# risc0/paritytech-bn

Hardware: AMD Instinct MI355X
Metric: BN254 pairings/sec (batched) at 1/2/4/8 MI355X; bit-exact vs CPU ref (higher is better)
Workload: dtype u32 (9x29-bit Montgomery digits, integer only)

## Files before the change

include/bn254mi.h:

```cpp
#ifndef BN254MI_H
#define BN254MI_H
#include <stddef.h>
#include <stdint.h>

#ifdef __cplusplus
extern "C" {
#endif

typedef struct { uint64_t l[4]; } bn_fq;
typedef struct { bn_fq c0, c1; } bn_fq2;
typedef struct { uint64_t l[4]; } bn_fr;
typedef struct { bn_fq x, y, z; } bn_g1;
typedef struct { bn_fq2 x, y, z; } bn_g2;
typedef struct { bn_fq c[12]; } bn_gt;

typedef enum {
    BN_OK = 0,
    BN_ERR_INVALID_ARGUMENT = 1,
    BN_ERR_TO_AFFINE = 2,
    BN_ERR_FE_ZERO = 3,
    BN_ERR_HIP = 4,
    BN_ERR_NO_DEVICE = 5,
    BN_ERR_INTERNAL = 6
} bn_status;
// ... 89 lines not shown

int bn_fq_from_slice_many(bn_ctx* ctx, const uint8_t* be32, size_t n, bn_fq* out, uint8_t* status);
int bn_fq_to_big_endian_many(bn_ctx* ctx, const bn_fq* a, size_t n, uint8_t* be32);
int bn_fq2_from_slice_many(bn_ctx* ctx, const uint8_t* be64, size_t n, bn_fq2* out, uint8_t* status);
int bn_fr_from_slice_many(bn_ctx* ctx, const uint8_t* be32, size_t n, bn_fr* out);
int bn_fr_to_big_endian_many(bn_ctx* ctx, const bn_fr* a, size_t n, uint8_t* be32);
int bn_fq_sqrt_many(bn_ctx* ctx, const bn_fq* a, size_t n, bn_fq* out, uint8_t* ok);
int bn_fq2_sqrt_many(bn_ctx* ctx, const bn_fq2* a, size_t n, bn_fq2* out, uint8_t* ok);
int bn_g1_affine_new_many(bn_ctx* ctx, const bn_fq* x, const bn_fq* y, size_t n, bn_g1* out, uint8_t* status);
int bn_g2_affine_new_many(bn_ctx* ctx, const bn_fq2* x, const bn_fq2* y, size_t n, bn_g2* out, uint8_t* status);
int bn_g2_affine_new_many_dev(bn_ctx* ctx, const bn_fq2* d_x, const bn_fq2* d_y, size_t n, bn_g2* d_out,
                              uint8_t* d_status, void* stream);
int bn_g1_from_compressed_many(bn_ctx* ctx, const uint8_t* b33, size_t n, bn_g1* out, uint8_t* status);
int bn_g2_from_compressed_many(bn_ctx* ctx, const uint8_t* b65, size_t n, bn_g2* out, uint8_t* status);
int bn_g1_from_compressed_many_dev(bn_ctx* ctx, const uint8_t* d_b33, size_t n, bn_g1* d_out, uint8_t* d_status,
                                   void* stream);
int bn_g2_from_compressed_many_dev(bn_ctx* ctx, const uint8_t* d_b65, size_t n, bn_g2* d_out, uint8_t* d_status,
                                   void* stream);
int bn_gt_pow_many(bn_ctx* ctx, const bn_gt* a, const bn_fr* k, size_t n, bn_gt* out);
int bn_gt_pow_many_dev(bn_ctx* ctx, const bn_gt* d_a, const bn_fr* d_k, size_t n, bn_gt* d_out, void* stream);

int bn_set_phase_timing(bn_ctx* ctx, int enable);
int bn_set_fe_wide_max(bn_ctx* ctx, size_t n);
int bn_set_latency_max(bn_ctx* ctx, size_t n);
int bn_get_phase_times(bn_ctx* ctx, float ms[4], int* launches);

size_t bn_workspace_bytes(size_t n);
int bn_reserve(bn_ctx* ctx, size_t n);

#ifdef __cplusplus
}
#endif
#endif
```

paritytech-bn_amd/csrc/capi.hip:

```cpp
#include <hip/hip_runtime.h>
#include <stdlib.h>
#include <string.h>

#include <algorithm>
#include <array>
#include <initializer_list>
#include <mutex>
#include <string>
#include <thread>
#include <vector>

#include "kernels.h"

using namespace bn;

#include "ctx.h"

namespace {

int fail(bn_ctx* c, int code, const std::string& msg) {
    if (c) c->err = msg;
    return code;
}
#define HIPCHK(ctx, x)                                                                   \
// ... 1153 lines not shown
        HIPCHK(c, hipGetLastError());
    }
    return BN_OK;
}
int bn_pairing_batch_dev(bn_ctx* c, const bn_g1* d_p, const bn_g2* d_q, size_t n, bn_gt* d_out, int* d_status,
                         void* stream) {
    CTX_GUARD(c);
    return batch_dev(c, d_p, d_q, n, d_out, d_status, 0, pick(c, stream));
}
int bn_miller_loop_batch_dev(bn_ctx* c, const bn_g2* d_q, const bn_g1* d_p, size_t n, bn_gt* d_out, int* d_status,
                             void* stream) {
    CTX_GUARD(c);
    return batch_dev(c, d_p, d_q, n, d_out, d_status, 1, pick(c, stream));
}
int bn_set_latency_max(bn_ctx* c, size_t n) {
    if (c && !c->subs.empty()) {
        for (bn_ctx* d : c->subs) RET_IF(bn_set_latency_max(d, n));
        return BN_OK;
    }
    CTX_GUARD(c);
    c->latency_max = n;
    return BN_OK;
}
int bn_set_fe_wide_max(bn_ctx* c, size_t n) {
    if (c && !c->subs.empty()) {
        for (bn_ctx* d : c->subs) RET_IF(bn_set_fe_wide_max(d, n));
        return BN_OK;
    }
    CTX_GUARD(c);
    c->fe_wide_max = n;
    return BN_OK;
}

int bn_final_exponentiation_many(bn_ctx* c, const bn_gt* f, size_t n, bn_gt* out, uint8_t* ok) {
    if (c && !c->subs.empty()) return bn_multi_final_exponentiation_many(c, f, n, out, ok);
    CTX_GUARD_HOST(c);
    if (n == 0) return BN_OK;
    if (!f || !out) return fail(c, BN_ERR_INVALID_ARGUMENT, "null buffer");
    RET_IF(clear_err(c, c->stream));
    int zero = 0;
    return final_exp_host(c, f, n, out, ok, &zero);
}

int bn_miller_loop_many(bn_ctx* c, const bn_g1* p, const bn_g2* q, size_t n, bn_gt* out) {
    if (c && !c->subs.empty()) return bn_multi_miller_loop_many(c, p, q, n, out);
    CTX_GUARD_HOST(c);
// ... 266 lines not shown
        bn_gt* dout = db + m;
        uint32_t* dprog = (uint32_t*)(dout + m);
        HIPCHK(c, hipMemcpyAsync(da, a + off, m * sizeof(bn_gt), hipMemcpyHostToDevice, c->stream));
        k_gt_load<<<grid_for(kPathLanes * m), kBlock, 0, c->stream>>>(da, m, c->slots + (size_t)1 * kSlotWords * m);
        if (op == BN_FQ12_MUL) {
            HIPCHK(c, hipMemcpyAsync(db, b + off, m * sizeof(bn_gt), hipMemcpyHostToDevice, c->stream));
            k_gt_load<<<grid_for(kPathLanes * m), kBlock, 0, c->stream>>>(db, m, c->slots + (size_t)2 * kSlotWords * m);
        }
        Prog P;
        P.next = 3;
        uint32_t res = P.tmp();
        switch (op) {
            case BN_FQ12_MUL: P.op(OP_MUL, res, 1, 2); break;
            case BN_FQ12_SQR: P.op(OP_SQR, res, 1); break;
            case BN_FQ12_INV: P.op(OP_INV, res, 1); break;
            case BN_FQ12_CYC_SQR: P.op(OP_CYC, res, 1); break;
            case BN_FQ12_EXP_BY_NEG_Z: res = P.exp_by_neg_z(1); break;
            case BN_FQ12_FROB1: P.op(OP_FROB1, res, 1); break;
            case BN_FQ12_FROB2: P.op(OP_FROB2, res, 1); break;
            default: P.op(OP_FROB3, res, 1); break;
        }
        P.finalize({res});
        HIPCHK(c, hipMemcpyAsync(dprog, P.s.data(), P.s.size() * 4, hipMemcpyHostToDevice, c->stream));
        k_fq12_vm<<<grid_pair(kPathLanes * m), kPairBlock, 0, c->stream>>>(dprog, P.steps(), c->slots, m);
        k_gt_store<<<grid_for(kPathLanes * m), kBlock, 0, c->stream>>>(c->slots + (size_t)res * kSlotWords * m, m, m, dout);
        HIPCHK(c, hipGetLastError());
        HIPCHK(c, hipMemcpyAsync(out + off, dout, m * sizeof(bn_gt), hipMemcpyDeviceToHost, c->stream));
        HIPCHK(c, hipStreamSynchronize(c->stream));
    }
    return BN_OK;
}

int bn_fq_from_slice_many(bn_ctx* c, const uint8_t* be32, size_t n, bn_fq* out, uint8_t* st) {
    CTX_GUARD_HOST(c);
    return staged(c, n, {{be32, 32}}, {{out, sizeof(bn_fq)}, {st, 1}}, [&](void** d, size_t m, hipStream_t s) -> int {
        KL(k_fq_from_slice, (const uint8_t*)d[0], m, (bn_fq*)d[1], (uint8_t*)d[2]);
        return BN_OK;
    });
}
int bn_fq_to_big_endian_many(bn_ctx* c, const bn_fq* a, size_t n, uint8_t* be32) {
    CTX_GUARD_HOST(c);
    return staged(c, n, {{a, sizeof(bn_fq)}}, {{be32, 32}}, [&](void** d, size_t m, hipStream_t s) -> int {
        KL(k_fq_to_be, (const bn_fq*)d[0], m, (uint8_t*)d[1]);
        return BN_OK;
    });
}
int bn_fq2_from_slice_many(bn_ctx* c, const uint8_t* be64, size_t n, bn_fq2* out, uint8_t* st) {
// ... 219 lines not shown
```

paritytech-bn_amd/csrc/ctx.h:

```cpp
#pragma once
#include <hip/hip_runtime.h>

#include <array>
#include <mutex>
#include <string>
#include <vector>

#include "../../include/bn254mi.h"

struct bn_ctx {
    int device = 0;
    hipStream_t stream = nullptr;
    std::mutex mu;
    std::mutex err_mu;
    std::string err;
    size_t cap = 0;
    uint32_t* coeffs = nullptr;
    uint32_t* paff = nullptr;
    uint32_t* slots = nullptr;
    uint8_t* flags = nullptr;
    uint32_t* d_prog = nullptr;
    bool timing = false;
    std::vector<hipEvent_t> ev_pool;
    std::vector<std::array<hipEvent_t, 5>> ev_marks;
    int fe_steps = 0;
    int fe_out = 0;
    bool fe_last_out = false;
    size_t fe_wide_max = 0;
    int miller_form = 3;
    size_t latency_max = 0;
    bool latency_w2 = true;
    size_t lat_w1_max = 2048;
    size_t prepare_wide_max = 0;
    int* d_err = nullptr;
    uint32_t* tail_ws = nullptr;
    uint32_t tail_epoch = 0;
    uint32_t* fe_ds_ws = nullptr;
    size_t fe_ds_max = 0;
    size_t stage_bytes = 0;
    void* stage = nullptr;
    int host_pipeline = 1;
    size_t host_piece = 0;
    size_t pin_bytes = 0;
    void* pin = nullptr;
    hipStream_t h2d = nullptr, d2h = nullptr;
    hipEvent_t ev_in[2] = {}, ev_comp[2] = {}, ev_out[2] = {};
    hipEvent_t ws_event = nullptr;
    bool ws_pending = false;
    int msm_window = 0;
    size_t msm_min = 0;
    uint32_t* msm_keys = nullptr;
// ... 29 lines not shown
```

paritytech-bn_amd/csrc/kernels.h:

```cpp
#pragma once
#include <hip/hip_runtime.h>

#include "../../include/bn254mi.h"
#include "pairing.h"
#include "msm.h"

namespace bn {

constexpr int kBlock = 256;
constexpr int kPathLanes = BN_PATH_SPLIT ? 2 : 1;
constexpr int kSlotLaneWords = BN_SPLIT ? 54 : 108;
#if BN_SPLIT
#define BN_PATH_ATTR __attribute__((amdgpu_waves_per_eu(2, 2)))
#else
#define BN_PATH_ATTR
#endif
constexpr int kCoeffFq = BN_NUM_COEFFS * 6;
constexpr size_t kChunk = size_t(1) << 18;
constexpr int kSlotWords = 108;
constexpr int kGtPowEntries = 17;
constexpr uint32_t kMsmSegment = 16;
constexpr int kMsmScanBlock = 1024;

template <int B>
// ... 403 lines not shown
__global__ void __launch_bounds__(kBlock) k_horner_wide(const uint32_t* __restrict__ g, size_t n, SegPlan plan,
                                                        int do_fe, bn_gt* __restrict__ out, int* __restrict__ err, int duo);
__global__ void __launch_bounds__(kBlock) k_horner_tree(const uint32_t* __restrict__ g, SegPlan plan, int do_fe,
                                                        bn_gt* __restrict__ out, int* __restrict__ err, int duo);
__global__ void __launch_bounds__(kPairBlock) k_prepare(const bn_g1* __restrict__ p, const bn_g2* __restrict__ q, size_t n,
                          uint32_t* __restrict__ coeffs, uint32_t* __restrict__ paff, uint8_t* __restrict__ flags,
                          int* __restrict__ err, int mode, int scale);
constexpr int kPrepareWideLanes = 8;
#ifndef BN_LINES_PRESCALED
#define BN_LINES_PRESCALED 1
#endif
__global__ void __launch_bounds__(kPairBlock) k_prepare_wide(const bn_g1* __restrict__ p, const bn_g2* __restrict__ q,
                                                         size_t n, uint32_t* __restrict__ coeffs,
                                                         uint32_t* __restrict__ paff, uint8_t* __restrict__ flags,
                                                         int* __restrict__ err, int mode, int scale);
__global__ void __launch_bounds__(kBlock) k_coeffs_store(const uint32_t* __restrict__ coeffs, size_t n,
                                                         bn_fq2* __restrict__ out);
__global__ void __launch_bounds__(kPairBlock) k_pairing_fused(const bn_g1* __restrict__ p, const bn_g2* __restrict__ q,
                                                          size_t n, uint8_t* __restrict__ flags, int* __restrict__ err,
                                                          int mode, uint32_t* __restrict__ f_out);
__global__ void __launch_bounds__(kBlock) k_miller(const uint32_t* __restrict__ coeffs, const uint32_t* __restrict__ paff,
                         const uint8_t* __restrict__ flags, size_t n, uint32_t* __restrict__ f_out);
__global__ void __launch_bounds__(kPairBlock) k_fq12_vm(const uint32_t* __restrict__ prog, int nsteps, uint32_t* slots, size_t n);
__global__ void __launch_bounds__(kPairBlock) k_pairing_full(const bn_g1* __restrict__ p, const bn_g2* __restrict__ q,
                                                          size_t n, const uint32_t* __restrict__ prog, int nsteps,
                                                          uint32_t* __restrict__ slots, bn_gt* __restrict__ out,
                                                          int* __restrict__ err);
__global__ void __launch_bounds__(kBlock) k_fe_out(const uint32_t* __restrict__ slots, size_t n, int out_slot, const uint8_t* __restrict__ flags,
                         bn_gt* __restrict__ out, uint8_t* __restrict__ ok, int* __restrict__ err);
__global__ void __launch_bounds__(kBlock) k_fe_wide(const uint32_t* __restrict__ f, size_t stride, size_t n,
                                                    bn_gt* __restrict__ out, uint8_t* __restrict__ ok,
                                                    int* __restrict__ err, int duo);
__global__ void __launch_bounds__(kBlock) k_fq12_reduce_wide(const uint32_t* __restrict__ in, size_t in_stride,
                                                             SetSpan sets, uint32_t* __restrict__ out,
                                                             size_t out_stride, size_t out_base, size_t out_set, int per_group);
constexpr int kTailBlock = 256;
__global__ void __launch_bounds__(kTailBlock) k_horner_tree2(const uint32_t* __restrict__ g, SegPlan plan, int do_fe,
                                                             bn_gt* __restrict__ out, int* __restrict__ err,
                                                             const uint32_t* __restrict__ zf);
constexpr int kTailChanWords = 1024 + 2 * 128 * 88;
__global__ void __launch_bounds__(kTailBlock) k_seg_fe1(uint32_t* __restrict__ g, SegPlan plan,
                                                        uint32_t* __restrict__ zf);
constexpr int kTailWsWords = kTailChanWords + 2 * kMaxSeg * 256;
__global__ void __launch_bounds__(kTailBlock) k_seg_tail(const uint32_t* __restrict__ g, SegPlan plan,
                                                         bn_gt* __restrict__ out, int* __restrict__ err,
                                                         uint32_t* __restrict__ ws, uint32_t epoch);
// ... 57 lines not shown
```

paritytech-bn_amd/csrc/kernels_pairing.hip:

```cpp
#ifndef BN_FOLD_LDS
#define BN_FOLD_LDS 1
#endif
#include "fq.h"
#define BN_SPLIT BN_PATH_SPLIT
#include "kernels.h"
#include "lines_wide.h"
#include "fe_vm.h"

namespace bn {

__global__ void BN_PATH_ATTR __launch_bounds__(kPairBlock) k_prepare(const bn_g1* __restrict__ p,
                                                                    const bn_g2* __restrict__ q, size_t n,
                                                                    uint32_t* __restrict__ coeffs,
                                                                    uint32_t* __restrict__ paff,
                                                                    uint8_t* __restrict__ flags,
                                                                    int* __restrict__ err, int mode, int scale) {
    fold_table_init();
    const Balance bal = balance_init();
    const size_t l = lane_id(), i = l / kL, nl = kL * n;
    if (i >= n) return;
    const PairAffine a = pair_to_affine(p, q, i, l, flags, err, mode);
    st_fq(paff, nl, l, 0, a.px);
    st_fq(paff, nl, l, 1, a.py);
    const bool sc = BN_LINES_PRESCALED && scale;
// ... 99 lines not shown
    const size_t l = lane_id(), i = l / kL, nl = kL * n;
    if (i >= n) return;
#pragma unroll 1
    for (int k = 0; k < BN_NUM_COEFFS; ++k)
#pragma unroll
        for (int j = 0; j < 3; ++j) st_ref2(out[(i * BN_NUM_COEFFS + k) * 3 + j], ld_fq2<kLine>(coeffs, nl, l, k * 6 + 2 * j));
}

__global__ void BN_PATH_ATTR __launch_bounds__(kPairBlock) k_pairing_fused(const bn_g1* __restrict__ p,
                                                                          const bn_g2* __restrict__ q, size_t n,
                                                                          uint8_t* __restrict__ flags,
                                                                          int* __restrict__ err, int mode,
                                                                          uint32_t* __restrict__ f_out) {
    fold_table_init();
    const Balance bal = balance_init();
    const size_t l = lane_id(), i = l / kL, nl = kL * n;
    if (i >= n) return;
    const PairAffine a = pair_to_affine(p, q, i, l, flags, err, mode);
    Fq12<kF> f = miller_fused(a.qa, a.px, a.py, [&](int d) { balance_step(bal, (uint32_t)d); });
    if (flags[l]) f = widen<kF>(fq12_one());
    st_fq12(f_out, nl, l, f);
}

__global__ void BN_PATH_ATTR __launch_bounds__(kPairBlock) k_pairing_full(const bn_g1* __restrict__ p,
                                                                         const bn_g2* __restrict__ q, size_t n,
                                                                         const uint32_t* __restrict__ prog, int nsteps,
                                                                         uint32_t* __restrict__ slots,
                                                                         bn_gt* __restrict__ out, int* __restrict__ err) {
    fold_table_init();
    const Balance bal = balance_init();
    const size_t l = lane_id(), i = l / kL, nl = kL * n;
    if (i >= n) return;
    const PairAffine a = pair_to_affine(p, q, i, l, nullptr, err, 0);
    Fq12<kF> f = miller_fused(a.qa, a.px, a.py, [&](int d) { balance_step(bal, (uint32_t)d); });
    if (a.skip) f = widen<kF>(fq12_one());
    const bool zero = !a.skip && fq12_is_zero(f);
    st_fq12(slots, nl, l, f);
    const Fq12<kF> r = fq12_vm_run(prog, nsteps, slots, nl, l, bal, 1u << 20, false);
    if (zero) {
        if ((l % kL) == 0) err_or(err, BN_ERR_FE_ZERO);
        st_gt_zero(out[i]);
    } else if (a.skip) {
        st_gt(out[i], fq12_one());
    } else {
        st_gt(out[i], r);
    }
// ... 141 lines not shown
```

paritytech-bn_amd/csrc/pairing.h:

```cpp
#pragma once
#include "curve.h"

namespace bn {

constexpr int kF = 2;
template <int S, int B>
BN_INLINE Fq12<S> narrow12(const Fq12<B>& a) {
    if constexpr (kv(B) <= S) {
        return widen<S>(fq12_norm(a));
    } else {
        return widen<S>(fq12_fold(a));
    }
}

template <int B, typename Emit>
BN_INLINE void g2_precompute(const G2Aff<B>& q, Emit&& emit) {
    G2Proj r = {widen<kPt>(q.x), widen<kPt>(q.y), widen<kPt>(fq2_one())};
    const G2Aff<B> q_neg = {q.x, fq2_neg(q.y)};
    int k = 0;
#pragma unroll 1
    for (int i = 0; i < BN_NAF_DIGITS; ++i) {
        emit(k++, doubling_step(r));
        if ((kNafNonzero >> i) & 1u) {
            const bool minus = (kNafMinus >> i) & 1u;
            G2Aff<B> base = {q.x, fq2_select(minus, q_neg.y, q.y)};
            emit(k++, mixed_addition_step(r, base));
        }
    }
    G2Aff<kPt> q1 = mul_by_q(q);
    G2Aff<kPt> q2 = mul_by_q(q1);
    q2.y = fq2_neg(q2.y);
    emit(k++, mixed_addition_step(r, q1));
    emit(k++, mixed_addition_step(r, q2));
}

#if BN_SPLIT
#ifndef BN_DOT6_ASM
#define BN_DOT6_ASM 1
#endif
struct LineOps {
    Fq<kLine> y;
    Fq<8> w;
};
template <int X>
BN_INLINE LineOps line_ops(const Fq2<X>& v_in) {
    const Fq<kv(X)> v = fq_norm(v_in.c);
    const bool odd = lane_odd();
#if defined(__HIP_DEVICE_COMPILE__)
    Fq<kjoin(kv(X), kenc(kv(X) + 1, 2))> w;
    dpp_sel_own_partner(w.v, v.v, fq_neg_lazy(v).v);
    (void)odd;
    return {widen<kLine>(fq_bcast_c0(v)), widen<8>(fq_norm(w))};
#else
    const Fq<kv(X)> pv = fq_partner(v);
    return {widen<kLine>(fq_select(odd, pv, v)), widen<8>(fq_norm(fq_pick(odd, v, fq_neg_lazy(pv))))};
#endif
}
BN_INLINE void acc_mad2(Acc& t, const Fq<2>& u, const LineOps& v) {
    acc_mad(t, u, v.y);
    acc_mad(t, fq_partner(u), v.w);
}
template <int F, int X>
BN_INLINE Fq12<2> fq12_mul_by_024_lazy(const Fq12<F>& f_in, const Fq2<X>& x0_in, const Fq2<X>& x4_in,
                                       const Fq2<X>& x2_in) {
    static_assert(kl(F) == 1 && kv(F) <= 2, "fq12_mul_by_024_lazy: f normalized, bound 2");
    const LineOps x0 = line_ops(x0_in), x4 = line_ops(x4_in), x2 = line_ops(x2_in);
    const Fq<2> f0 = widen<2>(f_in.c0.c0.c), f1 = widen<2>(f_in.c1.c0.c), f2 = widen<2>(f_in.c0.c1.c);
    const Fq<2> f3 = widen<2>(f_in.c1.c1.c), f4 = widen<2>(f_in.c0.c2.c), f5 = widen<2>(f_in.c1.c2.c);
    auto xi = [](const Fq<2>& u) { return fq2_fold(fq2_mul_xi(Fq2<2>{u})).c; };
    auto out = [&](const Fq<2>& a, const LineOps& va, const Fq<2>& b, const LineOps& vb, const Fq<2>& c,
                   const LineOps& vc) {
#if BN_DOT6_ASM && BN_DOT2_ASM && defined(__HIP_DEVICE_COMPILE__)
        const Fq<2> pa = fq_partner(a), pb = fq_partner(b), pc = fq_partner(c);
        Fq<2> r;
        asm(BN_ASM_DOT6 : BN_ASM_OUT9(r.v)
            : BN_ASM_IN9(a.v), BN_ASM_IN9(va.y.v), BN_ASM_IN9(pa.v), BN_ASM_IN9(va.w.v), BN_ASM_IN9(b.v),
              BN_ASM_IN9(vb.y.v), BN_ASM_IN9(pb.v), BN_ASM_IN9(vb.w.v), BN_ASM_IN9(c.v), BN_ASM_IN9(vc.y.v),
              BN_ASM_IN9(pc.v), BN_ASM_IN9(vc.w.v), BN_ASM_P
            : BN_ASM_CLOBBER);
        return Fq2<2>{r};
#else
        Acc t = {};
        acc_mad2(t, a, va);
        acc_mad2(t, b, vb);
        acc_mad2(t, c, vc);
        return Fq2<2>{acc_redc<2>(t)};
#endif
    };
    const Fq2<2> o5 = out(f5, x0, f2, x4, f1, x2);
    const Fq2<2> o4 = out(f4, x0, f1, x4, f0, x2);
    const Fq<2> g5 = xi(f5);
    const Fq2<2> o3 = out(f3, x0, f0, x4, g5, x2);
    const Fq<2> g4 = xi(f4);
    const Fq2<2> o2 = out(f2, x0, g5, x4, g4, x2);
    const Fq<2> g3 = xi(f3);
    const Fq2<2> o1 = out(f1, x0, g4, x4, g3, x2);
    const Fq<2> g2 = xi(f2);
    const Fq2<2> o0 = out(f0, x0, g3, x4, g2, x2);
    return {{o0, o2, o4}, {o1, o3, o5}};
}
#endif

template <int B, int PB>
BN_INLINE Fq12<kF> apply_line(const Fq12<B>& f, const Ell& c, const Fq<PB>& px, const Fq<PB>& py) {
#if BN_SPLIT
    return widen<kF>(fq12_mul_by_024_lazy(narrow12<2>(f), c.ell_0, narrow<kLine>(fq2_scale(c.ell_vw, py)),
                                          narrow<kLine>(fq2_scale(c.ell_vv, px))));
#else
    return narrow12<kF>(fq12_mul_by_024(f, c.ell_0, narrow<kLine>(fq2_scale(c.ell_vw, py)),
                                        narrow<kLine>(fq2_scale(c.ell_vv, px))));
// ... 147 lines not shown
```

paritytech-bn_amd/csrc/tower.h:

```cpp
#pragma once
#include "fq.h"


namespace bn {

constexpr int cmax(int a, int b) { return a > b ? a : b; }

constexpr int kInvRounds = 19;
constexpr Limbs9 kR3 = {{0x0e2312b2u, 0x16c05ca2u, 0x0bc84389u, 0x1cdf310bu, 0x11adafddu, 0x032e568eu, 0x1d6ae48cu,
                         0x10d4cd1fu, 0x0026c2d2u}};
BN_INLINE uint32_t bgcd_lin_exact(const uint32_t (&x)[9], const uint32_t (&y)[9], int32_t f, int32_t g,
                                  uint32_t (&r)[9]) {
    int64_t c = 0;
#pragma unroll
    for (int i = 0; i < 9; ++i) {
        const int64_t t = (int64_t)(int32_t)x[i] * f + (int64_t)(int32_t)y[i] * g + c;
        if (i) r[i - 1] = (uint32_t)t & M29;
        c = t >> 29;
    }
    r[8] = (uint32_t)c;
    const uint32_t m = (uint32_t)((int32_t)r[8] >> 31);
    int64_t cn = 0;
#pragma unroll
    for (int i = 0; i < 8; ++i) {
// ... 507 lines not shown
}
template <int L, int B>
BN_INLINE auto pre(const Fq6<B>& a) {
    if constexpr (kv(B) <= L) return a; else return fq6_fold(a);
}
template <int B>
BN_INLINE auto fq6_mul_by_nonresidue(const Fq6<B>& a) { return mk6(fq2_mul_xi(a.c2), a.c0, a.c1); }

template <int A, int B>
BN_INLINE auto fq6_mul(const Fq6<A>& a, const Fq6<B>& b) {
    if constexpr (kv(A) > 20 || kv(B) > 20) return fq6_mul(pre<20>(a), pre<20>(b)); else {
    const auto p1 = fq2_mul2(a.c0, b.c0, a.c1, b.c1);
    const auto& a_a = p1.a;
    const auto& b_b = p1.b;
    const auto p2 = fq2_mul2(a.c2, b.c2, fq2_add(a.c1, a.c2), fq2_add(b.c1, b.c2));
    const auto& c_c = p2.a;
    auto t0 = fq2_sub(fq2_sub(p2.b, b_b), c_c);
    const auto p3 = fq2_mul2(fq2_add(a.c0, a.c1), fq2_add(b.c0, b.c1), fq2_add(a.c0, a.c2), fq2_add(b.c0, b.c2));
    auto t1 = fq2_sub(fq2_sub(p3.a, a_a), b_b);
    auto t2 = fq2_sub(p3.b, a_a);
    return mk6(fq2_add(fq2_mul_xi(t0), a_a), fq2_add(t1, fq2_mul_xi(c_c)), fq2_sub(fq2_add(t2, b_b), c_c));
    }
}
template <int A>
BN_INLINE auto fq6_sqr(const Fq6<A>& a) {
    if constexpr (kv(A) > 20) return fq6_sqr(fq6_fold(a)); else {
    auto s0 = fq2_sqr(a.c0);
    auto s1 = fq2_dbl(fq2_mul(a.c0, a.c1));
    auto s2 = fq2_sqr(fq2_add(fq2_sub(a.c0, a.c1), a.c2));
    auto s3 = fq2_dbl(fq2_mul(a.c1, a.c2));
    auto s4 = fq2_sqr(a.c2);
    return mk6(fq2_add(s0, fq2_mul_xi(s3)), fq2_add(s1, fq2_mul_xi(s4)),
               fq2_sub(fq2_sub(fq2_add(fq2_add(s1, s2), s3), s0), s4));
    }
}
template <int B>
BN_INLINE auto fq6_inv(const Fq6<B>& a_in) {
    auto a = fq6_fold(a_in);
    auto c0 = fq2_fold(fq2_sub(fq2_sqr(a.c0), fq2_mul(a.c1, fq2_mul_xi(a.c2))));
    auto c1 = fq2_fold(fq2_sub(fq2_mul_xi(fq2_sqr(a.c2)), fq2_mul(a.c0, a.c1)));
    auto c2 = fq2_fold(fq2_sub(fq2_sqr(a.c1), fq2_mul(a.c0, a.c2)));
    auto t = fq2_inv(fq2_fold(fq2_add(fq2_mul_xi(fq2_add(fq2_mul(a.c2, c1), fq2_mul(a.c1, c2))), fq2_mul(a.c0, c0))));
    return mk6(fq2_mul(t, c0), fq2_mul(t, c1), fq2_mul(t, c2));
}

BN_INLINE Fq2<1> fq6_frob_c1(int n) {
// ... 29 lines not shown
BN_INLINE Fq12<1> fq12_one() { return {fq6_one(), fq6_zero()}; }
template <int B>
BN_INLINE Fq12<2> fq12_fold(const Fq12<B>& a) { return {fq6_fold(a.c0), fq6_fold(a.c1)}; }
template <int B>
BN_INLINE Fq12<kv(B)> fq12_norm(const Fq12<B>& a) { return {fq6_norm(a.c0), fq6_norm(a.c1)}; }
template <int B>
BN_INLINE bool fq12_is_zero(const Fq12<B>& a) { return ((unsigned)fq6_is_zero(a.c0) & (unsigned)fq6_is_zero(a.c1)) != 0; }
template <int L, int B>
BN_INLINE auto pre(const Fq12<B>& a) {
    if constexpr (kv(B) <= L) return a; else return fq12_fold(a);
}
template <int B>
BN_INLINE auto fq12_conj(const Fq12<B>& a) { return mk12(a.c0, fq6_neg(a.c1)); }
template <int A, int B>
BN_INLINE auto fq12_add(const Fq12<A>& a, const Fq12<B>& b) { return mk12(fq6_add(a.c0, b.c0), fq6_add(a.c1, b.c1)); }
template <int A, int B>
BN_INLINE auto fq12_sub(const Fq12<A>& a, const Fq12<B>& b) { return mk12(fq6_sub(a.c0, b.c0), fq6_sub(a.c1, b.c1)); }
template <int B>
BN_INLINE auto fq12_neg(const Fq12<B>& a) { return mk12(fq6_neg(a.c0), fq6_neg(a.c1)); }

template <int A, int B>
BN_INLINE auto fq12_mul(const Fq12<A>& a, const Fq12<B>& b) {
    if constexpr (kv(A) > 10 || kv(B) > 10) return fq12_mul(pre<10>(a), pre<10>(b)); else {
    auto aa = fq6_fold(fq6_mul(a.c0, b.c0));
    auto bb = fq6_fold(fq6_mul(a.c1, b.c1));
    auto t = fq6_mul(fq6_add(a.c0, a.c1), fq6_add(b.c0, b.c1));
    return mk12(fq6_add(fq6_mul_by_nonresidue(bb), aa), fq6_sub(fq6_sub(t, aa), bb));
    }
}
template <int A>
BN_INLINE auto fq12_sqr(const Fq12<A>& a) {
    if constexpr (kv(A) > 2) return fq12_sqr(fq12_fold(a)); else {
    auto ab = fq6_fold(fq6_mul(a.c0, a.c1));
    auto t = fq6_mul(fq6_add(fq6_mul_by_nonresidue(a.c1), a.c0), fq6_add(a.c0, a.c1));
    return mk12(fq6_sub(fq6_sub(t, ab), fq6_mul_by_nonresidue(ab)), fq6_add(ab, ab));
    }
}
template <int B>
BN_INLINE auto fq12_inv(const Fq12<B>& a_in) {
    auto a = fq12_fold(a_in);
    auto t = fq6_inv(fq6_sub(fq6_fold(fq6_sqr(a.c0)), fq6_mul_by_nonresidue(fq6_fold(fq6_sqr(a.c1)))));
    return mk12(fq6_mul(a.c0, t), fq6_neg(fq6_mul(a.c1, t)));
}
template <int POWER, int B>
BN_INLINE auto fq12_frobenius_map(const Fq12<B>& a) {
    auto c1 = fq6_frobenius_map<POWER>(a.c1);
    if constexpr (POWER == 2) {
        const Fq<1> k = fq_from_limbs<1>(Limbs9{BN_FQ12_C1_2_C0});
        return mk12(fq6_frobenius_map<POWER>(a.c0), mk6(fq2_scale(c1.c0, k), fq2_scale(c1.c1, k), fq2_scale(c1.c2, k)));
    } else {
        Fq2<1> k = fq12_frob_c1(POWER);
        return mk12(fq6_frobenius_map<POWER>(a.c0), mk6(fq2_mul(c1.c0, k), fq2_mul(c1.c1, k), fq2_mul(c1.c2, k)));
    }
}

template <int F, int X>
BN_INLINE auto fq12_mul_by_024(const Fq12<F>& f, const Fq2<X>& ell_0, const Fq2<X>& ell_vw, const Fq2<X>& ell_vv) {
// ... 115 lines not shown
```

paritytech-bn_amd/substrate_bn/_native.py:

```python
import ctypes
import os

import numpy as np

PKG_DIR = os.path.dirname(os.path.dirname(os.path.abspath(__file__)))
LIB_PATH = os.environ.get("BN254MI_LIB") or os.path.join(PKG_DIR, "libbn254mi.so")

BN_OK = 0
BN_ERR_INVALID_ARGUMENT = 1
BN_ERR_TO_AFFINE = 2
BN_ERR_FE_ZERO = 3
BN_ERR_HIP = 4
BN_ERR_NO_DEVICE = 5
BN_ERR_INTERNAL = 6

FQ12_OPS = {"mul": 0, "sqr": 1, "inv": 2, "cyc_sqr": 3, "exp_by_neg_z": 4, "frob1": 5, "frob2": 6, "frob3": 7}

EXPORTS = [
    "bn_ctx_create", "bn_ctx_destroy", "bn_last_error", "bn_ctx_stream",
    "bn_pairing_many", "bn_pairing_many_dev", "bn_pairing_batch", "bn_miller_loop_batch",
    "bn_final_exponentiation_many", "bn_miller_loop_many",
    "bn_g1_mul_many", "bn_g1_mul_many_dev", "bn_g2_mul_many", "bn_g2_mul_many_dev",
    "bn_fq12_op_many", "bn_workspace_bytes", "bn_reserve", "bn_set_phase_timing", "bn_get_phase_times",
    "bn_fq_from_slice_many", "bn_fq_to_big_endian_many", "bn_fq2_from_slice_many", "bn_fr_from_slice_many",
    "bn_fr_to_big_endian_many", "bn_fq_sqrt_many", "bn_fq2_sqrt_many", "bn_g1_affine_new_many",
    "bn_g2_affine_new_many", "bn_g2_affine_new_many_dev", "bn_g1_from_compressed_many", "bn_g2_from_compressed_many",
    "bn_g1_from_compressed_many_dev", "bn_g2_from_compressed_many_dev", "bn_gt_pow_many", "bn_gt_pow_many_dev",
    "bn_ctx_create_multi", "bn_ctx_num_devices", "bn_ctx_device", "bn_shard_range", "bn_pairing_many_allgather_dev",
    "bn_pairing_batch_dev", "bn_miller_loop_batch_dev", "bn_set_fe_wide_max", "bn_g2_precompute_many",
    "bn_set_latency_max", "bn_dev_status",
    "bn_g1_msm", "bn_g1_msm_dev", "bn_set_msm_window", "bn_set_msm_min", "bn_msm_reserve",
] + ["bn_%s_%s_many%s" % (g, op, dev) for g in ("g1", "g2") for op in ("add", "sub", "neg", "normalize", "eq")
     for dev in ("", "_dev")]
GROUP_OPS = ("add", "sub", "neg", "normalize", "eq")

ST_OK, ST_FIELD_INVALID_SLICE_LENGTH, ST_FIELD_INVALID_U512, ST_FIELD_NOT_MEMBER = 0, 1, 2, 3
ST_CURVE_INVALID_ENCODING, ST_CURVE_NOT_MEMBER, ST_GROUP_NOT_ON_CURVE, ST_GROUP_NOT_IN_SUBGROUP = 4, 5, 6, 7


class BnError(RuntimeError):
    def __init__(self, code, msg):
        super().__init__("bn254mi error %d: %s" % (code, msg))
        self.code = code


_lib = None


def load():
    global _lib
    if _lib is not None:
        return _lib
    if not os.path.exists(LIB_PATH):
# ... 30 lines not shown
        "bn_fq2_from_slice_many": ([vp, vp, sz, vp, vp], i),
        "bn_fr_from_slice_many": ([vp, vp, sz, vp], i),
        "bn_fr_to_big_endian_many": ([vp, vp, sz, vp], i),
        "bn_fq_sqrt_many": ([vp, vp, sz, vp, vp], i),
        "bn_fq2_sqrt_many": ([vp, vp, sz, vp, vp], i),
        "bn_g1_affine_new_many": ([vp, vp, vp, sz, vp, vp], i),
        "bn_g2_affine_new_many": ([vp, vp, vp, sz, vp, vp], i),
        "bn_g2_affine_new_many_dev": ([vp, vp, vp, sz, vp, vp, vp], i),
        "bn_g1_from_compressed_many": ([vp, vp, sz, vp, vp], i),
        "bn_g2_from_compressed_many": ([vp, vp, sz, vp, vp], i),
        "bn_g1_from_compressed_many_dev": ([vp, vp, sz, vp, vp, vp], i),
        "bn_g2_from_compressed_many_dev": ([vp, vp, sz, vp, vp, vp], i),
        "bn_gt_pow_many": ([vp, vp, vp, sz, vp], i),
        "bn_gt_pow_many_dev": ([vp, vp, vp, sz, vp, vp], i),
        "bn_ctx_create_multi": ([vp, i, ctypes.POINTER(vp)], i),
        "bn_ctx_num_devices": ([vp], i),
        "bn_ctx_device": ([vp, i], vp),
        "bn_shard_range": ([sz, i, i, ctypes.POINTER(sz), ctypes.POINTER(sz)], None),
        "bn_pairing_many_allgather_dev": ([vp, vp, vp, sz, vp, vp], i),
        "bn_pairing_batch_dev": ([vp, vp, vp, sz, vp, vp, vp], i),
        "bn_miller_loop_batch_dev": ([vp, vp, vp, sz, vp, vp, vp], i),
        "bn_set_fe_wide_max": ([vp, sz], i),
        "bn_set_latency_max": ([vp, sz], i),
        "bn_g2_precompute_many": ([vp, vp, sz, vp], i),
        "bn_dev_status": ([vp, vp], i),
        "bn_g1_msm": ([vp, vp, vp, sz, vp], i),
        "bn_g1_msm_dev": ([vp, vp, vp, sz, vp, vp], i),
        "bn_set_msm_window": ([vp, i], i),
        "bn_set_msm_min": ([vp, sz], i),
        "bn_msm_reserve": ([vp, sz], i),
    }
    for g in ("g1", "g2"):
        for op in GROUP_OPS:
            unary = op in ("neg", "normalize")
            sig["bn_%s_%s_many" % (g, op)] = ([vp, vp, sz, vp] if unary else [vp, vp, vp, sz, vp], i)
            sig["bn_%s_%s_many_dev" % (g, op)] = ([vp, vp, sz, vp, vp] if unary else [vp, vp, vp, sz, vp, vp], i)
    ab_build = bool(os.environ.get("BN254MI_LIB"))
    for name, (args, res) in sig.items():
        if ab_build and not hasattr(L, name):
            continue
        fn = getattr(L, name)
        fn.argtypes = args
        fn.restype = res
    _lib = L
    return L

# ... 191 lines not shown
        self._check(self._L.bn_g2_mul_many_dev(self._h, d_p, d_k, n, d_out, stream))

    def g1_msm_dev(self, d_p, d_k, n, d_out, stream=None):
        self._check(self._L.bn_g1_msm_dev(self._h, d_p, d_k, n, d_out, stream))

    def set_msm_window(self, c):
        self._check(self._L.bn_set_msm_window(self._h, c))

    def set_msm_min(self, n):
        self._check(self._L.bn_set_msm_min(self._h, n))

    def msm_reserve(self, n):
        self._check(self._L.bn_msm_reserve(self._h, n))

    def pairing_batch_dev(self, d_p, d_q, n, d_out, d_status=None, stream=None):
        self._check(self._L.bn_pairing_batch_dev(self._h, d_p, d_q, n, d_out, d_status, stream))

    def miller_loop_batch_dev(self, d_q, d_p, n, d_out, d_status=None, stream=None):
        self._check(self._L.bn_miller_loop_batch_dev(self._h, d_q, d_p, n, d_out, d_status, stream))

    def set_fe_wide_max(self, n):
        self._check(self._L.bn_set_fe_wide_max(self._h, n))

    def set_latency_max(self, n):
        self._check(self._L.bn_set_latency_max(self._h, n))

    def set_phase_timing(self, enable=True):
        self._check(self._L.bn_set_phase_timing(self._h, 1 if enable else 0))

    def phase_times(self):
        ms = np.zeros(4, np.float32)
        cnt = np.zeros(1, np.int32)
        self._check(self._L.bn_get_phase_times(self._h, _ptr(ms), _ptr(cnt)))
        return ms.astype(float), int(cnt[0])

    def _bytes_in(self, b, width):
        b = np.ascontiguousarray(b, dtype=np.uint8)
        if b.size % width:
            raise ValueError("byte buffer of %d is not a multiple of %d" % (b.size, width))
        return b.reshape(-1, width)

    def fq_from_slice_many(self, be32):
        b = self._bytes_in(be32, 32)
        out = np.zeros((b.shape[0], 4), np.uint64)
        st = np.zeros(b.shape[0], np.uint8)
        self._check(self._L.bn_fq_from_slice_many(self._h, _ptr(b), b.shape[0], _ptr(out), _ptr(st)))
# ... 97 lines not shown
```

Baseline: 9.174 million.

## Add lazy Fq6 multiplication via dot6 line-op products for Fq12 mul/sqr

Introduces a lazy Fq6 product that precomputes partner and xi-scaled digits of one operand and forms each output coefficient with a single fused 6-term dot product and one Montgomery reduction. Fq12 mul and sqr in the pairing compilation unit use it by default (BN_FQ6_LAZY=3), replacing the Karatsuba Fq6 multiply with fold steps. The aim is fewer reductions and folds per Fq12 op in the Miller loop and final exponentiation, at the cost of more register pressure from the precomputed operands. It also adds an opt-in pairing-path VM kernel for the fq12 op API, which is off by default.

```diff
diff --git a/include/bn254mi.h b/include/bn254mi.h
--- a/include/bn254mi.h
+++ b/include/bn254mi.h
@@ -135,6 +135,7 @@
 
 int bn_set_phase_timing(bn_ctx* ctx, int enable);
 int bn_set_fe_wide_max(bn_ctx* ctx, size_t n);
+int bn_set_fq12_op_unit(bn_ctx* ctx, int unit);
 int bn_set_latency_max(bn_ctx* ctx, size_t n);
 int bn_get_phase_times(bn_ctx* ctx, float ms[4], int* launches);
 
diff --git a/paritytech-bn_amd/csrc/capi.hip b/paritytech-bn_amd/csrc/capi.hip
--- a/paritytech-bn_amd/csrc/capi.hip
+++ b/paritytech-bn_amd/csrc/capi.hip
@@ -1199,6 +1199,16 @@
     c->latency_max = n;
     return BN_OK;
 }
+int bn_set_fq12_op_unit(bn_ctx* c, int unit) {
+    if (c && !c->subs.empty()) {
+        for (bn_ctx* d : c->subs) RET_IF(bn_set_fq12_op_unit(d, unit));
+        return BN_OK;
+    }
+    CTX_GUARD(c);
+    if (unit != 0 && unit != 1) return fail(c, BN_ERR_INVALID_ARGUMENT, "unit must be 0 or 1");
+    c->fq12_op_unit = unit;
+    return BN_OK;
+}
 int bn_set_fe_wide_max(bn_ctx* c, size_t n) {
     if (c && !c->subs.empty()) {
         for (bn_ctx* d : c->subs) RET_IF(bn_set_fe_wide_max(d, n));
@@ -1511,7 +1521,10 @@
         }
         P.finalize({res});
         HIPCHK(c, hipMemcpyAsync(dprog, P.s.data(), P.s.size() * 4, hipMemcpyHostToDevice, c->stream));
-        k_fq12_vm<<<grid_pair(kPathLanes * m), kPairBlock, 0, c->stream>>>(dprog, P.steps(), c->slots, m);
+        if (c->fq12_op_unit == 1)
+            k_fq12_vm_pairing<<<grid_pair(kPathLanes * m), kPairBlock, 0, c->stream>>>(dprog, P.steps(), c->slots, m);
+        else
+            k_fq12_vm<<<grid_pair(kPathLanes * m), kPairBlock, 0, c->stream>>>(dprog, P.steps(), c->slots, m);
         k_gt_store<<<grid_for(kPathLanes * m), kBlock, 0, c->stream>>>(c->slots + (size_t)res * kSlotWords * m, m, m, dout);
         HIPCHK(c, hipGetLastError());
         HIPCHK(c, hipMemcpyAsync(out + off, dout, m * sizeof(bn_gt), hipMemcpyDeviceToHost, c->stream));
diff --git a/paritytech-bn_amd/csrc/ctx.h b/paritytech-bn_amd/csrc/ctx.h
--- a/paritytech-bn_amd/csrc/ctx.h
+++ b/paritytech-bn_amd/csrc/ctx.h
@@ -27,6 +27,7 @@
     int fe_out = 0;
     bool fe_last_out = false;
     size_t fe_wide_max = 0;
+    int fq12_op_unit = 0;
     int miller_form = 3;
     size_t latency_max = 0;
     bool latency_w2 = true;
diff --git a/paritytech-bn_amd/csrc/kernels.h b/paritytech-bn_amd/csrc/kernels.h
--- a/paritytech-bn_amd/csrc/kernels.h
+++ b/paritytech-bn_amd/csrc/kernels.h
@@ -449,6 +449,7 @@
 __global__ void __launch_bounds__(kBlock) k_miller(const uint32_t* __restrict__ coeffs, const uint32_t* __restrict__ paff,
                          const uint8_t* __restrict__ flags, size_t n, uint32_t* __restrict__ f_out);
 __global__ void __launch_bounds__(kPairBlock) k_fq12_vm(const uint32_t* __restrict__ prog, int nsteps, uint32_t* slots, size_t n);
+__global__ void __launch_bounds__(kPairBlock) k_fq12_vm_pairing(const uint32_t* __restrict__ prog, int nsteps, uint32_t* slots, size_t n);
 __global__ void __launch_bounds__(kPairBlock) k_pairing_full(const bn_g1* __restrict__ p, const bn_g2* __restrict__ q,
                                                           size_t n, const uint32_t* __restrict__ prog, int nsteps,
                                                           uint32_t* __restrict__ slots, bn_gt* __restrict__ out,
diff --git a/paritytech-bn_amd/csrc/kernels_pairing.hip b/paritytech-bn_amd/csrc/kernels_pairing.hip
--- a/paritytech-bn_amd/csrc/kernels_pairing.hip
+++ b/paritytech-bn_amd/csrc/kernels_pairing.hip
@@ -1,5 +1,15 @@
 #ifndef BN_FOLD_LDS
 #define BN_FOLD_LDS 1
+#endif
+#ifndef BN_FQ6_LAZY
+#define BN_FQ6_LAZY 3
+#endif
+#ifndef BN_CYC_LIN
+#if BN_FQ6_LAZY == 3
+#define BN_CYC_LIN 7
+#else
+#define BN_CYC_LIN 0
+#endif
 #endif
 #include "fq.h"
 #define BN_SPLIT BN_PATH_SPLIT
@@ -145,6 +155,15 @@
     st_fq12(f_out, nl, l, f);
 }
 
+__global__ void BN_PATH_ATTR __launch_bounds__(kPairBlock) k_fq12_vm_pairing(const uint32_t* __restrict__ prog,
+                                                                            int nsteps, uint32_t* slots, size_t n) {
+    fold_table_init();
+    const Balance bal = balance_init();
+    const size_t i = lane_id();
+    if (i >= kL * n) return;
+    (void)fq12_vm_run(prog, nsteps, slots, kL * n, i, bal, 0, true);
+}
+
 __global__ void BN_PATH_ATTR __launch_bounds__(kPairBlock) k_pairing_full(const bn_g1* __restrict__ p,
                                                                          const bn_g2* __restrict__ q, size_t n,
                                                                          const uint32_t* __restrict__ prog, int nsteps,
diff --git a/paritytech-bn_amd/csrc/pairing.h b/paritytech-bn_amd/csrc/pairing.h
--- a/paritytech-bn_amd/csrc/pairing.h
+++ b/paritytech-bn_amd/csrc/pairing.h
@@ -35,30 +35,11 @@
 }
 
 #if BN_SPLIT
-#ifndef BN_DOT6_ASM
-#define BN_DOT6_ASM 1
-#endif
-struct LineOps {
-    Fq<kLine> y;
-    Fq<8> w;
-};
+using LineOps = LineOpsT<kLine, kLine + 1>;
 template <int X>
 BN_INLINE LineOps line_ops(const Fq2<X>& v_in) {
-    const Fq<kv(X)> v = fq_norm(v_in.c);
-    const bool odd = lane_odd();
-#if defined(__HIP_DEVICE_COMPILE__)
-    Fq<kjoin(kv(X), kenc(kv(X) + 1, 2))> w;
-    dpp_sel_own_partner(w.v, v.v, fq_neg_lazy(v).v);
-    (void)odd;
-    return {widen<kLine>(fq_bcast_c0(v)), widen<8>(fq_norm(w))};
-#else
-    const Fq<kv(X)> pv = fq_partner(v);
-    return {widen<kLine>(fq_select(odd, pv, v)), widen<8>(fq_norm(fq_pick(odd, v, fq_neg_lazy(pv))))};
-#endif
-}
-BN_INLINE void acc_mad2(Acc& t, const Fq<2>& u, const LineOps& v) {
-    acc_mad(t, u, v.y);
-    acc_mad(t, fq_partner(u), v.w);
+    const auto o = line_ops_of(v_in);
+    return {widen<kLine>(o.y), widen<kLine + 1>(o.w)};
 }
 template <int F, int X>
 BN_INLINE Fq12<2> fq12_mul_by_024_lazy(const Fq12<F>& f_in, const Fq2<X>& x0_in, const Fq2<X>& x4_in,
@@ -70,22 +51,7 @@
     auto xi = [](const Fq<2>& u) { return fq2_fold(fq2_mul_xi(Fq2<2>{u})).c; };
     auto out = [&](const Fq<2>& a, const LineOps& va, const Fq<2>& b, const LineOps& vb, const Fq<2>& c,
                    const LineOps& vc) {
-#if BN_DOT6_ASM && BN_DOT2_ASM && defined(__HIP_DEVICE_COMPILE__)
-        const Fq<2> pa = fq_partner(a), pb = fq_partner(b), pc = fq_partner(c);
-        Fq<2> r;
-        asm(BN_ASM_DOT6 : BN_ASM_OUT9(r.v)
-            : BN_ASM_IN9(a.v), BN_ASM_IN9(va.y.v), BN_ASM_IN9(pa.v), BN_ASM_IN9(va.w.v), BN_ASM_IN9(b.v),
-              BN_ASM_IN9(vb.y.v), BN_ASM_IN9(pb.v), BN_ASM_IN9(vb.w.v), BN_ASM_IN9(c.v), BN_ASM_IN9(vc.y.v),
-              BN_ASM_IN9(pc.v), BN_ASM_IN9(vc.w.v), BN_ASM_P
-            : BN_ASM_CLOBBER);
-        return Fq2<2>{r};
-#else
-        Acc t = {};
-        acc_mad2(t, a, va);
-        acc_mad2(t, b, vb);
-        acc_mad2(t, c, vc);
-        return Fq2<2>{acc_redc<2>(t)};
-#endif
+        return Fq2<2>{fq_dot6(a, va, b, vb, c, vc)};
     };
     const Fq2<2> o5 = out(f5, x0, f2, x4, f1, x2);
     const Fq2<2> o4 = out(f4, x0, f1, x4, f0, x2);
diff --git a/paritytech-bn_amd/csrc/tower.h b/paritytech-bn_amd/csrc/tower.h
--- a/paritytech-bn_amd/csrc/tower.h
+++ b/paritytech-bn_amd/csrc/tower.h
@@ -553,6 +553,109 @@
     return mk6(fq2_add(fq2_mul_xi(t0), a_a), fq2_add(t1, fq2_mul_xi(c_c)), fq2_sub(fq2_add(t2, b_b), c_c));
     }
 }
+#if BN_SPLIT
+template <int Y, int W>
+struct LineOpsT {
+    Fq<Y> y;
+    Fq<W> w;
+};
+template <int X>
+BN_INLINE LineOpsT<kv(X), kv(X) + 1> line_ops_of(const Fq2<X>& v_in) {
+    const Fq<kv(X)> v = fq_norm(v_in.c);
+    const bool odd = lane_odd();
+#if defined(__HIP_DEVICE_COMPILE__)
+    Fq<kjoin(kv(X), kenc(kv(X) + 1, 2))> w;
+    dpp_sel_own_partner(w.v, v.v, fq_neg_lazy(v).v);
+    (void)odd;
+    return {fq_bcast_c0(v), fq_norm(w)};
+#else
+    const Fq<kv(X)> pv = fq_partner(v);
+    return {fq_select(odd, pv, v), fq_norm(fq_pick(odd, v, fq_neg_lazy(pv)))};
+#endif
+}
+#ifndef BN_DOT6_ASM
+#define BN_DOT6_ASM 1
+#endif
+template <int A, int B, int C, int YA, int WA, int YB, int WB, int YC, int WC>
+BN_INLINE auto fq_dot6p(const Fq<A>& a, const Fq<A>& pa, const LineOpsT<YA, WA>& va, const Fq<B>& b, const Fq<B>& pb,
+                        const LineOpsT<YB, WB>& vb, const Fq<C>& c, const Fq<C>& pc, const LineOpsT<YC, WC>& vc) {
+    static_assert(kl(A) == 1 && kl(B) == 1 && kl(C) == 1, "fq_dot6: normalized u-side digits");
+    static_assert(kl(YA) == 1 && kl(WA) == 1 && kl(YB) == 1 && kl(WB) == 1 && kl(YC) == 1 && kl(WC) == 1,
+                  "fq_dot6: normalized v-side digits");
+    constexpr long long S = (long long)kv(A) * (kv(YA) + kv(WA)) + (long long)kv(B) * (kv(YB) + kv(WB)) +
+                            (long long)kv(C) * (kv(YC) + kv(WC));
+    constexpr int BO = 1 + (int)(S * 5908 / 1000000 + 1);
+    static_assert(BO <= kMaxBound, "fq_dot6: the value must stay below 2^261");
+    static_assert(S > 54 || BO == 2, "fq_dot6: the sparse line product's contract leaves below 2 p");
+#if BN_DOT6_ASM && BN_DOT2_ASM && defined(__HIP_DEVICE_COMPILE__)
+    Fq<BO> r;
+    asm(BN_ASM_DOT6 : BN_ASM_OUT9(r.v)
+        : BN_ASM_IN9(a.v), BN_ASM_IN9(va.y.v), BN_ASM_IN9(pa.v), BN_ASM_IN9(va.w.v), BN_ASM_IN9(b.v),
+          BN_ASM_IN9(vb.y.v), BN_ASM_IN9(pb.v), BN_ASM_IN9(vb.w.v), BN_ASM_IN9(c.v), BN_ASM_IN9(vc.y.v),
+          BN_ASM_IN9(pc.v), BN_ASM_IN9(vc.w.v), BN_ASM_P
+        : BN_ASM_CLOBBER);
+    return r;
+#else
+    Acc t = {};
+    acc_mad(t, a, va.y);
+    acc_mad(t, pa, va.w);
+    acc_mad(t, b, vb.y);
+    acc_mad(t, pb, vb.w);
+    acc_mad(t, c, vc.y);
+    acc_mad(t, pc, vc.w);
+    return acc_redc<BO>(t);
+#endif
+}
+template <int A, int B, int C, int YA, int WA, int YB, int WB, int YC, int WC>
+BN_INLINE auto fq_dot6(const Fq<A>& a, const LineOpsT<YA, WA>& va, const Fq<B>& b, const LineOpsT<YB, WB>& vb,
+                       const Fq<C>& c, const LineOpsT<YC, WC>& vc) {
+    const Fq<A> pa = fq_partner(a);
+    const Fq<B> pb = fq_partner(b);
+    const Fq<C> pc = fq_partner(c);
+    return fq_dot6p(a, pa, va, b, pb, vb, c, pc, vc);
+}
+
+#ifndef BN_FQ6_LAZY
+#define BN_FQ6_LAZY 0
+#endif
+template <int U>
+struct Fq6U {
+    static constexpr int kG = 10 * kv(U) + 1;
+    Fq<U> u0, u1, u2, p0, p1, p2;
+    Fq<kG> g1, g2, q1, q2;
+};
+template <int U>
+BN_INLINE Fq<10 * kv(U) + 1> fq_xi_lin(const Fq<U>& own, const Fq<U>& par) {
+    static_assert(kl(U) == 1, "fq_xi_lin: normalized");
+    return fq_lin<9, 1>(own, fq_pick(lane_odd(), par, fq_neg_lazy(par)));
+}
+constexpr int kLazyIn = 4;
+template <int A>
+BN_INLINE auto fq6_lazy_u(const Fq6<A>& a_in) {
+    const auto a = fq6_norm(pre<kLazyIn>(a_in));
+    constexpr int U = decltype(a.c0.c)::kK;
+    Fq6U<U> r;
+    r.u0 = a.c0.c, r.u1 = a.c1.c, r.u2 = a.c2.c;
+    r.p0 = fq_partner(r.u0), r.p1 = fq_partner(r.u1), r.p2 = fq_partner(r.u2);
+    r.g1 = fq_xi_lin(r.u1, r.p1), r.g2 = fq_xi_lin(r.u2, r.p2);
+    r.q1 = fq_partner(r.g1), r.q2 = fq_partner(r.g2);
+    return r;
+}
+template <int U, int Y0, int W0, int Y1, int W1, int Y2, int W2>
+BN_INLINE auto fq6_mul_uv(const Fq6U<U>& a, const LineOpsT<Y0, W0>& v0, const LineOpsT<Y1, W1>& v1,
+                          const LineOpsT<Y2, W2>& v2) {
+    const auto c2 = fq_dot6p(a.u0, a.p0, v2, a.u1, a.p1, v1, a.u2, a.p2, v0);
+    const auto c1 = fq_dot6p(a.u0, a.p0, v1, a.u1, a.p1, v0, a.g2, a.q2, v2);
+    const auto c0 = fq_dot6p(a.u0, a.p0, v0, a.g1, a.q1, v2, a.g2, a.q2, v1);
+    return mk6(wrap2(c0), wrap2(c1), wrap2(c2));
+}
+template <int A, int B>
+BN_INLINE auto fq6_mul_lazy(const Fq6<A>& a, const Fq6<B>& b_in) {
+    const auto b = pre<kLazyIn>(b_in);
+    return fq6_mul_uv(fq6_lazy_u(a), line_ops_of(b.c0), line_ops_of(b.c1), line_ops_of(b.c2));
+}
+#endif
+
 template <int A>
 BN_INLINE auto fq6_sqr(const Fq6<A>& a) {
     if constexpr (kv(A) > 20) return fq6_sqr(fq6_fold(a)); else {
@@ -628,17 +731,30 @@
 template <int A, int B>
 BN_INLINE auto fq12_mul(const Fq12<A>& a, const Fq12<B>& b) {
     if constexpr (kv(A) > 10 || kv(B) > 10) return fq12_mul(pre<10>(a), pre<10>(b)); else {
+#if BN_SPLIT && (BN_FQ6_LAZY & 1)
+    auto aa = fq6_mul_lazy(a.c0, b.c0);
+    auto bb = fq6_mul_lazy(a.c1, b.c1);
+    auto t = fq6_mul_lazy(fq6_add(a.c0, a.c1), fq6_add(b.c0, b.c1));
+#else
     auto aa = fq6_fold(fq6_mul(a.c0, b.c0));
     auto bb = fq6_fold(fq6_mul(a.c1, b.c1));
     auto t = fq6_mul(fq6_add(a.c0, a.c1), fq6_add(b.c0, b.c1));
+#endif
     return mk12(fq6_add(fq6_mul_by_nonresidue(bb), aa), fq6_sub(fq6_sub(t, aa), bb));
     }
 }
 template <int A>
 BN_INLINE auto fq12_sqr(const Fq12<A>& a) {
     if constexpr (kv(A) > 2) return fq12_sqr(fq12_fold(a)); else {
+#if BN_SPLIT && (BN_FQ6_LAZY & 2)
+    const auto u1 = fq6_lazy_u(a.c1);
+    auto ab = fq6_mul_uv(u1, line_ops_of(a.c0.c0), line_ops_of(a.c0.c1), line_ops_of(a.c0.c2));
+    auto t = fq6_mul_uv(fq6_lazy_u(fq6_add(a.c0, a.c1)), line_ops_of(fq2_add(wrap2(u1.g2), a.c0.c0)),
+                        line_ops_of(fq2_add(a.c1.c0, a.c0.c1)), line_ops_of(fq2_add(a.c1.c1, a.c0.c2)));
+#else
     auto ab = fq6_fold(fq6_mul(a.c0, a.c1));
     auto t = fq6_mul(fq6_add(fq6_mul_by_nonresidue(a.c1), a.c0), fq6_add(a.c0, a.c1));
+#endif
     return mk12(fq6_sub(fq6_sub(t, ab), fq6_mul_by_nonresidue(ab)), fq6_add(ab, ab));
     }
 }
diff --git a/paritytech-bn_amd/substrate_bn/_native.py b/paritytech-bn_amd/substrate_bn/_native.py
--- a/paritytech-bn_amd/substrate_bn/_native.py
+++ b/paritytech-bn_amd/substrate_bn/_native.py
@@ -28,7 +28,7 @@
     "bn_g1_from_compressed_many_dev", "bn_g2_from_compressed_many_dev", "bn_gt_pow_many", "bn_gt_pow_many_dev",
     "bn_ctx_create_multi", "bn_ctx_num_devices", "bn_ctx_device", "bn_shard_range", "bn_pairing_many_allgather_dev",
     "bn_pairing_batch_dev", "bn_miller_loop_batch_dev", "bn_set_fe_wide_max", "bn_g2_precompute_many",
-    "bn_set_latency_max", "bn_dev_status",
+    "bn_set_latency_max", "bn_dev_status", "bn_set_fq12_op_unit",
     "bn_g1_msm", "bn_g1_msm_dev", "bn_set_msm_window", "bn_set_msm_min", "bn_msm_reserve",
 ] + ["bn_%s_%s_many%s" % (g, op, dev) for g in ("g1", "g2") for op in ("add", "sub", "neg", "normalize", "eq")
      for dev in ("", "_dev")]
@@ -105,6 +105,7 @@
         "bn_miller_loop_batch_dev": ([vp, vp, vp, sz, vp, vp, vp], i),
         "bn_set_fe_wide_max": ([vp, sz], i),
         "bn_set_latency_max": ([vp, sz], i),
+        "bn_set_fq12_op_unit": ([vp, i], i),
         "bn_g2_precompute_many": ([vp, vp, sz, vp], i),
         "bn_dev_status": ([vp, vp], i),
         "bn_g1_msm": ([vp, vp, vp, sz, vp], i),
@@ -342,6 +343,9 @@
     def set_fe_wide_max(self, n):
         self._check(self._L.bn_set_fe_wide_max(self._h, n))
 
+    def set_fq12_op_unit(self, unit):
+        self._check(self._L.bn_set_fq12_op_unit(self._h, unit))
+
     def set_latency_max(self, n):
         self._check(self._L.bn_set_latency_max(self._h, n))
 
```

Result: faster. 9.348 million, median of 6 (+1.9%).
